# hsp-iit/online-detection

Measured on AMD Instinct MI355X. Metric: FALKON fit+infer samples/sec (N=1e6 D=1024 M=1e4), higher is better.
Workload: dtype f32-accurate K_nM (X Z' as a two-term f16 split on the f16 MFMA, f32 accumulate) stored as 24-bit fixed point (step 2^-24) + f64 solver (preconditioner: K_MM, T and T^-1 in f64; the products of the A factor, which only preconditions, at f32 accuracy on the f16 MFMA)

## Files before the change

### include/odx.h

```cpp
#ifndef ODX_H
#define ODX_H
#include <stdint.h>
#ifdef __cplusplus
extern "C" {
#endif

#define ODX_OK 0
#define ODX_ERR_INVALID (-1)
#define ODX_ERR_HIP (-2)
#define ODX_ERR_UNSUPPORTED (-3)
#define ODX_ERR_WORKSPACE (-4)

typedef void* odx_stream_t;

const char* odx_last_error_string(void);
int odx_version(void);
int odx_device_cus(void);
int odx_set_option(const char* name, int value);
int odx_get_option(const char* name, int* value);
int odx_option_default(const char* name, int* value);
int odx_release_helper_streams(void);
int odx_set_helper_streams(odx_stream_t s0, odx_stream_t s1);
int odx_stream_create_cu_mask(const uint32_t* mask, int words, odx_stream_t* stream);
int odx_stream_destroy(odx_stream_t stream);
// ... 112 lines not shown
                                  void* workspace, int64_t workspace_bytes, odx_stream_t stream);
int64_t odx_knm_fwd_bwd_q_workspace_bytes(int64_t n, int64_t M, int fmt);
int odx_knm_fwd_bwd_q(const void* K, int64_t ldk, const void* Klo, int64_t ldlo, int fmt, int64_t n, int64_t M,
                      const double* v, const double* w, double* out, void* workspace, int64_t workspace_bytes,
                      odx_stream_t stream);
int64_t odx_knm_fwd_bwd2_q_workspace_bytes(int64_t n, int64_t M, int fmt);
int odx_knm_fwd_bwd2_q(const void* K, int64_t ldk, const void* Klo, int64_t ldlo, int fmt, int64_t n, int64_t M,
                       const double* v, const double* v2, double* out, double* out2, void* workspace,
                       int64_t workspace_bytes, odx_stream_t stream);
int odx_knm_fwd_bwd_q_t(const void* K, int64_t ldk, const void* Klo, int64_t ldlo, int fmt, int64_t n, int64_t M,
                        const double* v, const double* w, double* out, double* t_out, void* workspace,
                        int64_t workspace_bytes, odx_stream_t stream);
int odx_knm_fwd_bwd2_q_t(const void* K, int64_t ldk, const void* Klo, int64_t ldlo, int fmt, int64_t n, int64_t M,
                         const double* v, const double* v2, double* out, double* out2, double* t_out, void* workspace,
                         int64_t workspace_bytes, odx_stream_t stream);
int odx_knm_fwd_bwd_q_cols_t(const void* K, int64_t ldk, const void* Klo, int64_t ldlo, int fmt, int64_t n, int64_t M,
                             const double* v, const double* w, double* out, double* t_out, void* workspace,
                             int64_t workspace_bytes, int64_t Mv, const int32_t* col_of, const int32_t* start,
                             const int32_t* pos, odx_stream_t stream);
int odx_knm_fwd_bwd2_q_cols_t(const void* K, int64_t ldk, const void* Klo, int64_t ldlo, int fmt, int64_t n, int64_t M,
                              const double* v, const double* v2, double* out, double* out2, double* t_out, void* workspace,
                              int64_t workspace_bytes, int64_t Mv, const int32_t* col_of, const int32_t* start,
                              const int32_t* pos, odx_stream_t stream);
int odx_cols_fold_f64(const double* v, int64_t Mv, const int32_t* start, const int32_t* pos, int64_t M, double* out,
                      odx_stream_t stream);
int odx_cols_expand_f64(const double* x, int64_t M, const int32_t* col_of, int64_t Mv, double* out, odx_stream_t stream);
int64_t odx_knm_fwd_bwdn_q_workspace_bytes(int64_t n, int64_t M, int fmt, int nv);
int odx_knm_fwd_bwdn_q(const void* K, int64_t ldk, const void* Klo, int64_t ldlo, int fmt, int64_t n, int64_t M, int nv,
                       const double* V, int64_t ldv, double* out, int64_t ldo, void* workspace, int64_t workspace_bytes,
                       odx_stream_t stream);
int64_t odx_knm_fwd_bwdn_q_rw_workspace_bytes(int64_t n, int64_t M, int fmt, int nv);
int odx_knm_fwd_bwdn_q_rw(const void* K, int64_t ldk, const void* Klo, int64_t ldlo, int fmt, int64_t n, int64_t M, int nv,
                          const double* V, int64_t ldv, const double* D, int64_t ldd, const int32_t* wrow, double* out,
                          int64_t ldo, double* T_out, int64_t ldt, void* workspace, int64_t workspace_bytes,
                          odx_stream_t stream);
int64_t odx_knm_bwdn_q_workspace_bytes(int64_t n, int64_t M, int fmt, int nv);
int odx_knm_bwdn_q(const void* K, int64_t ldk, const void* Klo, int64_t ldlo, int fmt, int64_t n, int64_t M, int nv,
                   const double* W, int64_t ldw, double* out, int64_t ldo, void* workspace, int64_t workspace_bytes,
                   odx_stream_t stream);
int64_t odx_knm_fwdn_q_workspace_bytes(int64_t n, int64_t M, int fmt, int nv);
int odx_knm_fwdn_q(const void* K, int64_t ldk, const void* Klo, int64_t ldlo, int fmt, int64_t n, int64_t M, int nv,
                   const double* V, int64_t ldv, double* T, int64_t ldt, void* workspace, int64_t workspace_bytes,
                   odx_stream_t stream);
int odx_knm_mv(const void* K, int64_t ldk, const void* Klo, int64_t ldlo, int fmt, int64_t n, int64_t M, const double* alpha,
               float* out, int64_t ldo, odx_stream_t stream);
int64_t odx_gauss_ktk_stream_h2_rows(int64_t M, int D);
// ... 263 lines not shown
```

### online-detection_amd/csrc/knm_pass_q.hip

```cpp
#include <algorithm>
#include <stdlib.h>

#include "odx_internal.h"
#include "knm_q.h"

namespace odx {

template <int NT, int CH, int R, int NV, int FMT, int WPE>
__device__ __forceinline__ void knm_passq_body(const unsigned short* __restrict__ Khi, int64_t ldk,
                                               const unsigned char* __restrict__ Klo, int64_t ldlo, int64_t n,
                                               int64_t M, const double* __restrict__ v1, const double* __restrict__ v2,
                                               const double* __restrict__ w, double* __restrict__ slab, int64_t slab_ld,
                                               double* __restrict__ t_out, int wg, int nwg, int64_t Mv = 0,
                                               const int* __restrict__ cstart = nullptr, const int* __restrict__ cpos = nullptr) {
  constexpr int NW = NT / 64;
  constexpr int CW = QCW;
  extern __shared__ __attribute__((aligned(16))) double vsq[];
  __shared__ double red[2][NW][NV * R];
  const int tid = threadIdx.x, lane = tid & 63, wave = tid >> 6;
  const int nchunk = (int)((M + CW - 1) / CW);
  const int vcap = (nchunk + 1) * CW;
  const int64_t nblk = (n + R - 1) / R;
  const double vscale = FMT == QF_U24 ? 5.9604644775390625e-08 : 1.0;
  for (int i = tid; i < vcap; i += NT) {
// ... 156 lines not shown
  knm_passq_body<NT, CH, R, NV, FMT, WPE>(Khi, ldk, Klo, ldlo, n, M, v1, v2, w, slab, slab_ld, t_out, (int)blockIdx.x, (int)gridDim.x, Mv,
                                          cstart, cpos);
}

struct PassBatchQ {
  const unsigned short* Khi[ODX_MAX_ZBATCH];
  const unsigned char* Klo[ODX_MAX_ZBATCH];
  int64_t ldk[ODX_MAX_ZBATCH];
  int64_t ldlo[ODX_MAX_ZBATCH];
  int64_t n[ODX_MAX_ZBATCH];
  int M[ODX_MAX_ZBATCH];
  int grid[ODX_MAX_ZBATCH];
};

template <int NT, int CH, int R, int FMT, int WPE = (NT >= 1024 ? 4 : 2)>
__global__ __launch_bounds__(NT, WPE) void knm_passq_batched_kernel(PassBatchQ pb, const double* __restrict__ v, int64_t vstride,
                                                                    double* __restrict__ slab, int64_t slab_ld, int64_t slab_stride) {
  const int b = blockIdx.y;
  if ((int)blockIdx.x >= pb.grid[b]) return;
  knm_passq_body<NT, CH, R, 1, FMT, WPE>(pb.Khi[b], pb.ldk[b], pb.Klo[b], pb.ldlo[b], pb.n[b], pb.M[b], v + (int64_t)b * vstride, nullptr,
                                         nullptr, slab + (int64_t)b * slab_stride, slab_ld, nullptr, (int)blockIdx.x, pb.grid[b]);
}

template <int CH, int R, int FMT>
__device__ __forceinline__ void knm_passq_stag_body(const unsigned short* __restrict__ Khi, int64_t ldk,
                                                    const unsigned char* __restrict__ Klo, int64_t ldlo, int64_t n,
                                                    int64_t M, const double* __restrict__ v1,
                                                    const double* __restrict__ w, double* __restrict__ slab,
                                                    int64_t slab_ld, double* __restrict__ t_out, int wg, int nwg,
                                                    int64_t Mv = 0, const int* __restrict__ cstart = nullptr,
                                                    const int* __restrict__ cpos = nullptr) {
  constexpr int NT = 256, CW = QCW;
  extern __shared__ __attribute__((aligned(16))) double vsq[];
  __shared__ double red[2][2][4][R];
  const int tid = threadIdx.x, lane = tid & 63;
  const int h = __builtin_amdgcn_readfirstlane(tid >> 8), hw = __builtin_amdgcn_readfirstlane((tid >> 6) & 3);
  const int ht = tid & 255;
  const int nchunk = (int)((M + CW - 1) / CW);
  constexpr int vcap = CH * NT * CW;
  const int64_t nblk = (n + R - 1) / R;
  const double vscale = FMT == QF_U24 ? 5.9604644775390625e-08 : 1.0;
  for (int i = tid; i < vcap; i += 512) vsq[i] = (v1 != nullptr && i < M) ? q_v_entry(v1, i, Mv, cstart, cpos) * vscale : 0.0;
  const int voff_hi = ht * (2 * CW), voff_lo = ht * CW;
  double acc[CH][CW];
#pragma unroll
  for (int c = 0; c < CH; ++c)
#pragma unroll
    for (int e = 0; e < CW; ++e) acc[c][e] = 0.0;
  QChunk<FMT, CW> kr[R][CH];
  const int rowb_hi = (int)ldk * 2, rowb_lo = (int)ldlo;
  __amdgpu_buffer_rsrc_t rs_hi, rs_lo;
  int rows_open = R;
  auto open_block = [&](int64_t blk) {
    const int64_t row0 = blk * R;
    rows_open = (int)(n - row0 < R ? n - row0 : R);
    rs_hi = __builtin_amdgcn_make_buffer_rsrc(const_cast<unsigned short*>(Khi + row0 * ldk), (short)0, rows_open * rowb_hi, 0x00020000);
    if (FMT == QF_U24)
      rs_lo = __builtin_amdgcn_make_buffer_rsrc(const_cast<unsigned char*>(Klo + row0 * ldlo), (short)0, rows_open * rowb_lo, 0x00020000);
  };
  auto load_block = [&](int c) {
#pragma unroll
    for (int r = 0; r < R; ++r) {
      const int rr = r < rows_open ? r : rows_open - 1;
      const u32x2q th = __builtin_amdgcn_raw_buffer_load_b64(rs_hi, voff_hi, rr * rowb_hi + c * (NT * 2 * CW), 0);
      kr[r][c].hi[0] = th[0], kr[r][c].hi[1] = th[1];
      if (FMT == QF_U24) kr[r][c].lo[0] = __builtin_amdgcn_raw_buffer_load_b32(rs_lo, voff_lo, rr * rowb_lo + c * (NT * CW), 0);
    }
  };
  __shared__ unsigned int arrived[2];
  if (tid < 2) arrived[tid] = 0u;
  const int64_t first = 2 * (int64_t)wg + h, step = 2 * (int64_t)nwg;
// ... 53 lines not shown
      pp ^= 1;
#pragma unroll
      for (int c = 0; c < CH; ++c)
#pragma unroll
        for (int r = 0; r < R; ++r) {
          asm volatile("" : "+v"(kr[r][c].hi[0]));
          asm volatile("" : "+v"(kr[r][c].hi[1]));
          if (FMT == QF_U24) asm volatile("" : "+v"(kr[r][c].lo[0]));
        }
    }
    if (t_out != nullptr && hw == 0) {
      if (lane == 0) {
#pragma unroll
        for (int r = 0; r < R; ++r)
          if (blk * R + r < n) t_out[blk * R + r] = t[r];
      }
    }
#pragma unroll
    for (int r = 0; r < R; ++r) {
      const int64_t row = blk * R + r;
      if (row >= n) t[r] = 0.0;
      else if (w != nullptr) t[r] += w[row];
    }
    const bool more = k + 1 < mine;
    if (more) open_block(blk + step);
#pragma unroll
    for (int c = 0; c < CH; ++c) {
#pragma unroll
      for (int r = 0; r < R; ++r)
#pragma unroll
        for (int e = 0; e < CW; ++e) acc[c][e] = fma(q_entry<FMT, CW>(kr[r][c], e), t[r], acc[c][e]);
      load_block(c);
      __builtin_amdgcn_sched_barrier(0);
    }
  }
  double* my = slab + (2 * (int64_t)wg + h) * slab_ld;
#pragma unroll
  for (int c = 0; c < CH; ++c) {
    const int ch = ht + c * NT;
    if (ch < nchunk) {
#pragma unroll
      for (int e = 0; e < CW; ++e)
        if ((int64_t)ch * CW + e < slab_ld) my[(int64_t)ch * CW + e] = acc[c][e] * vscale;
    }
  }
}

template <int CH, int R, int FMT>
__global__ __launch_bounds__(512, 2) void knm_passq_stag_kernel(const unsigned short* __restrict__ Khi, int64_t ldk,
                                                                const unsigned char* __restrict__ Klo, int64_t ldlo, int64_t n,
                                                                int64_t M, const double* __restrict__ v1,
                                                                const double* __restrict__ w, double* __restrict__ slab,
                                                                int64_t slab_ld, double* __restrict__ t_out, int64_t Mv,
                                                                const int* __restrict__ cstart, const int* __restrict__ cpos) {
  knm_passq_stag_body<CH, R, FMT>(Khi, ldk, Klo, ldlo, n, M, v1, w, slab, slab_ld, t_out, (int)blockIdx.x, (int)gridDim.x, Mv, cstart, cpos);
}

template <int CH, int R, int FMT>
__global__ __launch_bounds__(512, 2) void knm_passq_stag_batched_kernel(PassBatchQ pb, const double* __restrict__ v, int64_t vstride,
                                                                        double* __restrict__ slab, int64_t slab_ld,
                                                                        int64_t slab_stride) {
  const int b = blockIdx.y;
  if ((int)blockIdx.x >= pb.grid[b]) return;
  knm_passq_stag_body<CH, R, FMT>(pb.Khi[b], pb.ldk[b], pb.Klo[b], pb.ldlo[b], pb.n[b], pb.M[b], v + (int64_t)b * vstride, nullptr,
                                  slab + (int64_t)b * slab_stride, slab_ld, nullptr, (int)blockIdx.x, pb.grid[b]);
}

struct QCfg {
  int nt, ch, r, wg_per_cu;
};

static bool pick_qcfg(int64_t M, int nv, int fmt, QCfg* cfg) {
  const int64_t chunks = (M + 3) / 4;
  if (nv == 1) {
    if (chunks <= 256) { *cfg = {256, 1, 16, 2}; return true; }
    if (chunks <= 512) { *cfg = {0, 2, 8, 2}; return true; }
    if (chunks <= 1024) { *cfg = {0, 4, 4, 2}; return true; }
    if (chunks <= 2048) { *cfg = {256, 8, 3, 2}; return true; }
    if (chunks <= 2560) { *cfg = {0, 10, 2, 1}; return true; }
    if (chunks <= 3072) { *cfg = {512, 6, 4, 1}; return true; }
    if (chunks <= 5110) { *cfg = {1024, 5, 1, 1}; return true; }
    return false;
  }
  if (chunks <= 1024 || chunks > 2560) return false;
  if (chunks <= 2048) *cfg = {512, 4, 2, 1};
  else *cfg = {512, 5, 2, 1};
  const int64_t lds = 2 * (chunks + 1) * 4 * 8 + 2 * (cfg->nt / 64) * cfg->r * 2 * 8 + 64;
  return lds <= 163840;
// ... 246 lines not shown
  ODX_PROPAGATE(require_workspace("odx_knm_fwd_bwd2_q", workspace, workspace_bytes, 2 * (int64_t)grid * slab_ld * (int64_t)sizeof(double)));
  double* slab = static_cast<double*>(workspace);
  const size_t lds = (size_t)(2 * (slab_ld + 4) * sizeof(double));
  ODX_PROPAGATE(q_dispatch(q_block(K, ldk, Klo, ldlo, fmt, n, M), [&](auto f, const QBlock& b) {
    return dispatch_passq<2, decltype(f)::value>(cfg, b, grid, lds, s, v, v2, nullptr, slab, slab_ld, t_out, cm);
  }));
  ODX_CHECK_LAUNCH("odx_knm_fwd_bwd2_q");
  if (cm.on()) return slab_reduce_cols_f64(slab, slab_ld, grid, 2, M, cm.Mv, cm.col_of, out, out2, s);
  return slab_reduce2_f64(slab, slab_ld, grid, M, out, out2, s);
}

extern "C" int odx_knm_fwd_bwd2_q(const void* K, int64_t ldk, const void* Klo, int64_t ldlo, int fmt, int64_t n, int64_t M,
                                  const double* v, const double* v2, double* out, double* out2, void* workspace,
                                  int64_t workspace_bytes, odx_stream_t stream) {
  return knm_fwd_bwd2_q_impl(K, ldk, Klo, ldlo, fmt, n, M, v, v2, out, out2, nullptr, workspace, workspace_bytes, stream);
}

extern "C" int odx_knm_fwd_bwd2_q_t(const void* K, int64_t ldk, const void* Klo, int64_t ldlo, int fmt, int64_t n, int64_t M,
                                    const double* v, const double* v2, double* out, double* out2, double* t_out, void* workspace,
                                    int64_t workspace_bytes, odx_stream_t stream) {
  return knm_fwd_bwd2_q_impl(K, ldk, Klo, ldlo, fmt, n, M, v, v2, out, out2, t_out, workspace, workspace_bytes, stream);
}

extern "C" int odx_knm_fwd_bwd_q_cols_t(const void* K, int64_t ldk, const void* Klo, int64_t ldlo, int fmt, int64_t n, int64_t M,
                                        const double* v, const double* w, double* out, double* t_out, void* workspace,
                                        int64_t workspace_bytes, int64_t Mv, const int32_t* col_of, const int32_t* start,
                                        const int32_t* pos, odx_stream_t stream) {
  ODX_REQUIRE(t_out == nullptr || v != nullptr, "odx_knm_fwd_bwd_q_cols_t: t_out needs v");
  const QCols cm = {Mv, col_of, start, pos};
  ODX_PROPAGATE(check_q_cols("odx_knm_fwd_bwd_q_cols_t", cm, M));
  return knm_fwd_bwd_q_impl(K, ldk, Klo, ldlo, fmt, n, M, v, w, out, t_out, workspace, workspace_bytes, stream, cm);
}

extern "C" int odx_knm_fwd_bwd2_q_cols_t(const void* K, int64_t ldk, const void* Klo, int64_t ldlo, int fmt, int64_t n, int64_t M,
                                         const double* v, const double* v2, double* out, double* out2, double* t_out,
                                         void* workspace, int64_t workspace_bytes, int64_t Mv, const int32_t* col_of,
                                         const int32_t* start, const int32_t* pos, odx_stream_t stream) {
  const QCols cm = {Mv, col_of, start, pos};
  ODX_PROPAGATE(check_q_cols("odx_knm_fwd_bwd2_q_cols_t", cm, M));
  return knm_fwd_bwd2_q_impl(K, ldk, Klo, ldlo, fmt, n, M, v, v2, out, out2, t_out, workspace, workspace_bytes, stream, cm);
}
```

### online-detection_amd/odx/hip.py

```python
import ctypes
import os

_LIB = None
_LIB_PATH = os.environ.get("ODX_LIB_PATH") or os.path.join(os.path.dirname(os.path.abspath(__file__)), "lib", "libodx.so")

ODX_OK = 0
KNM_F32, KNM_U24, KNM_BF16 = 0, 1, 2
KNM_CODE = {"f32": KNM_F32, "u24": KNM_U24, "bf16": KNM_BF16}
KERNEL_GAUSS, KERNEL_MATERN32, KERNEL_MATERN52 = 0, 1, 2
STREAM_MAX_VECTORS = 16
GRID_MAX_SIGMAS = 4
GEMM_LOWER_ONLY, GEMM_A_UPPER, GEMM_B_UPPER, GEMM_A_LOWER, GEMM_B_LOWER, GEMM_STORE_T = 1, 2, 4, 8, 16, 32


class OdxUnavailable(RuntimeError):
    pass


class OdxError(RuntimeError):
    pass


_vp, _i64, _i32, _f64, _f32 = ctypes.c_void_p, ctypes.c_int64, ctypes.c_int, ctypes.c_double, ctypes.c_float

# ... 61 lines not shown
                                 _i64, _vp]),
    "odx_falkon_cg_batched_workspace_bytes": (_i64, [_i32, _vp, _vp]),
    "odx_falkon_cg_batched_f64": (_i32, [_i32, _vp, _vp, _vp, _vp, _vp, _i64, _i64, _i64, _vp, _i64, _vp, _f64, _i32, _i32, _f64, _f64,
                                         _vp, _vp, _i64, _vp]),
    "odx_falkon_cg_batched_q_workspace_bytes": (_i64, [_i32, _vp, _vp, _i32]),
    "odx_falkon_cg_batched_q_f64": (_i32, [_i32, _vp, _vp, _vp, _vp, _i32, _vp, _vp, _vp, _i64, _i64, _i64, _vp, _i64, _vp, _f64, _i32, _i32,
                                           _f64, _f64, _vp, _vp, _i64, _vp]),
    "odx_knm_fwd_bwd_workspace_bytes": (_i64, [_i64, _i64]),
    "odx_set_pass_reserved_cus": (_i32, [_i32]),
    "odx_knm_fwd_bwd": (_i32, [_vp, _i64, _i64, _i64, _vp, _vp, _vp, _vp, _i64, _vp]),
    "odx_knm_fwd_bwd2_workspace_bytes": (_i64, [_i64, _i64]),
    "odx_knm_fwd_bwd2": (_i32, [_vp, _i64, _i64, _i64, _vp, _vp, _vp, _vp, _vp, _i64, _vp]),
    "odx_knm_ld": (_i64, [_i64, _i32]),
    "odx_knm_bytes": (_i64, [_i64, _i64, _i32]),
    "odx_gauss_knm_h2_store": (_i32, [_vp, _i64, _vp, _vp, _i64, _vp, _i64, _vp, _vp, _i64, _i32, _f64, _i32, _vp, _i64, _vp, _i64,
                                      _vp, _vp, _vp, _i64, _vp]),
    "odx_knm_fwd_bwd_t": (_i32, [_vp, _i64, _i64, _i64, _vp, _vp, _vp, _vp, _vp, _i64, _vp]),
    "odx_knm_fwd_bwd2_t": (_i32, [_vp, _i64, _i64, _i64, _vp, _vp, _vp, _vp, _vp, _vp, _i64, _vp]),
    "odx_knm_fwd_bwd_q_t": (_i32, [_vp, _i64, _vp, _i64, _i32, _i64, _i64, _vp, _vp, _vp, _vp, _vp, _i64, _vp]),
    "odx_knm_fwd_bwd2_q_t": (_i32, [_vp, _i64, _vp, _i64, _i32, _i64, _i64, _vp, _vp, _vp, _vp, _vp, _vp, _i64, _vp]),
    "odx_knm_fwd_bwd_q_cols_t": (_i32, [_vp, _i64, _vp, _i64, _i32, _i64, _i64, _vp, _vp, _vp, _vp, _vp, _i64, _i64, _vp, _vp, _vp, _vp]),
    "odx_knm_fwd_bwd2_q_cols_t": (_i32, [_vp, _i64, _vp, _i64, _i32, _i64, _i64, _vp, _vp, _vp, _vp, _vp, _vp, _i64, _i64, _vp, _vp, _vp,
                                         _vp]),
    "odx_cols_fold_f64": (_i32, [_vp, _i64, _vp, _vp, _i64, _vp, _vp]),
    "odx_cols_expand_f64": (_i32, [_vp, _i64, _vp, _i64, _vp, _vp]),
    "odx_cg_scores_axpy_f64": (_i32, [_vp, _vp, _vp, _i64, _vp]),
    "odx_cg_scores_store_f32": (_i32, [_vp, _i64, _vp, _i64, _vp]),
    "odx_knm_fwd_bwd_q_workspace_bytes": (_i64, [_i64, _i64, _i32]),
    "odx_knm_fwd_bwd_q": (_i32, [_vp, _i64, _vp, _i64, _i32, _i64, _i64, _vp, _vp, _vp, _vp, _i64, _vp]),
    "odx_knm_fwd_bwd2_q_workspace_bytes": (_i64, [_i64, _i64, _i32]),
    "odx_knm_fwd_bwd2_q": (_i32, [_vp, _i64, _vp, _i64, _i32, _i64, _i64, _vp, _vp, _vp, _vp, _vp, _i64, _vp]),
    "odx_knm_fwd_bwdn_q_workspace_bytes": (_i64, [_i64, _i64, _i32, _i32]),
    "odx_knm_fwd_bwdn_q": (_i32, [_vp, _i64, _vp, _i64, _i32, _i64, _i64, _i32, _vp, _i64, _vp, _i64, _vp, _i64, _vp]),
    "odx_knm_fwd_bwdn_q_rw_workspace_bytes": (_i64, [_i64, _i64, _i32, _i32]),
    "odx_knm_fwd_bwdn_q_rw": (_i32, [_vp, _i64, _vp, _i64, _i32, _i64, _i64, _i32, _vp, _i64, _vp, _i64, _vp, _vp, _i64, _vp, _i64,
                                     _vp, _i64, _vp]),
    "odx_knm_bwdn_q_workspace_bytes": (_i64, [_i64, _i64, _i32, _i32]),
    "odx_knm_bwdn_q": (_i32, [_vp, _i64, _vp, _i64, _i32, _i64, _i64, _i32, _vp, _i64, _vp, _i64, _vp, _i64, _vp]),
    "odx_knm_fwdn_q_workspace_bytes": (_i64, [_i64, _i64, _i32, _i32]),
    "odx_knm_fwdn_q": (_i32, [_vp, _i64, _vp, _i64, _i32, _i64, _i64, _i32, _vp, _i64, _vp, _i64, _vp, _i64, _vp]),
    "odx_knm_mv": (_i32, [_vp, _i64, _vp, _i64, _i32, _i64, _i64, _vp, _vp, _i64, _vp]),
    "odx_gauss_ktk_stream_h2_rows": (_i64, [_i64, _i32]),
    "odx_gauss_ktk_stream_h2_workspace_bytes": (_i64, [_i64, _i64, _i32]),
    "odx_gauss_ktk_stream_h2": (_i32, [_vp, _i64, _vp, _vp, _i64, _vp, _i64, _vp, _vp, _i64, _i32, _f64, _vp, _vp, _vp, _vp, _vp, _vp,
                                       _i64, _vp]),
    "odx_gauss_ktk_stream_h2n_rows": (_i64, [_i64, _i32]),
# ... 134 lines not shown
```

### online-detection_amd/odx/knm_path.py

```python
import ctypes

import torch

from . import hip


def _p(t):
    return ctypes.c_void_p(t.data_ptr()) if t is not None else ctypes.c_void_p(0)


def _compact(K):
    return K.fmt in hip.KNM_CODE and K.fmt != "f32"


def _qblock(K):
    return _p(K.K), K.ld, _p(K.lo), K.ld, hip.KNM_CODE[K.fmt]


def _mapped(K):
    return getattr(K, "cmap", None)


def _vlen(K):
    return K.Mv if _mapped(K) is not None else K.M
# ... 93 lines not shown
            return False
        return K.fmt == "stream" or self._ktk2_bytes(K) >= 0

    def ktk2(self, K, v1, v2, out1=None, out2=None, t_out=None):
        if t_out is not None:
            self._check_t_out(K, v1, t_out)
        if out1 is None:
            out1 = torch.empty(_vlen(K), dtype=torch.float64, device=self.device)
        if out2 is None:
            out2 = torch.empty(_vlen(K), dtype=torch.float64, device=self.device)
        if K.fmt == "stream":
            self._ktk_stream(K, v1, v2, None, out1, out2)
            return out1, out2
        vecs = (_p(v1), _p(v2), _p(out1), _p(out2), _p(t_out))
        if _compact(K) and _mapped(K) is not None:
            ws = self._pass_ws("ktk", "odx_knm_fwd_bwd2_q", K, hip.KNM_CODE[K.fmt])
            self._call("odx_knm_fwd_bwd2_q_cols_t", *_qblock(K), K.n, K.M, *vecs, _p(ws), ws.numel(), *_cols(K, self.device))
        elif _compact(K):
            ws = self._pass_ws("ktk", "odx_knm_fwd_bwd2_q", K, hip.KNM_CODE[K.fmt])
            self._call("odx_knm_fwd_bwd2_q_t", *_qblock(K), K.n, K.M, *vecs, _p(ws), ws.numel())
        else:
            ws = self._pass_ws("ktk", "odx_knm_fwd_bwd2", K)
            self._call("odx_knm_fwd_bwd2_t", *_fblock(K), K.n, K.M, *vecs, _p(ws), ws.numel())
        return out1, out2

    def _ktkn_bytes(self, K, nv):
        return self.lib.odx_knm_fwd_bwdn_q_workspace_bytes(max(K.n, 1), K.M, hip.KNM_CODE[K.fmt], nv)

    def ktkn_width(self, K):
        if _compact(K):
            for nv in (8, 4):
                if self._ktkn_bytes(K, nv) >= 0:
                    return nv
        return 2 if self.can_ktk2(K) else 1

    def ktkn_span(self, K):
        return hip.STREAM_MAX_VECTORS if K.fmt == "stream" else self.ktkn_width(K)

    def _ktkn_stream(self, K, V, out, l, g):
        F, Zf = K.F, K.Zf
        nbytes = self._pass_bytes("odx_gauss_ktk_stream_h2n", max(K.n, 1), K.M, F.D, g)
        ws = K.ring if K.ring is not None and K.ring.numel() >= nbytes else self._workspace("ktkn_stream", nbytes)
        self._call("odx_gauss_ktk_stream_h2n", _p(F.P), F.P.stride(0), _p(F.meta), _p(F.sq), K.n, _p(Zf.P), Zf.P.stride(0), _p(Zf.meta),
                   _p(Zf.sq), K.M, F.D, K.sigma, g, _p(V[l]), V.stride(0), _p(out[l]), out.stride(0), _p(ws), ws.numel())

    def _ktkn_plan(self, K, L):
# ... 223 lines not shown
```

### online-detection_amd/odx/solver.py

```python
import math
from dataclasses import dataclass

import torch


@dataclass
class SolverOptions:
    pc_epsilon: float = 1e-5
    cg_epsilon: float = 1e-7
    cg_tolerance: float = 1e-7
    cg_full_gradient_every: int = 10
    check_pivots: bool = True


_DEFERRED = None


class deferred_pivot_checks:

    def __enter__(self):
        global _DEFERRED
        self._prev, self.items = _DEFERRED, []
        _DEFERRED = self.items
        return self
# ... 56 lines not shown
class _Rows:

    def __init__(self, be, L, Mp, fold, send, recv):
        def mat():
            return be.zeros(L * Mp).view(L, Mp)
        self.B, self.X, self.R, self.Pv, self.AP, self.U, self.alpha = (mat() for _ in range(7))
        self.AX = mat() if fold else None
        self.v = (mat(), mat() if fold else None)
        self.send, self.recv = send, recv


def _slots(TT, CC, M, L=1, l=0):
    return [[(TT[j * L + l, :M], CC[j * L + l, :M]) for j in range(k)] for k in range(1, TT.shape[0] // L + 1)]


def _cg_state(be, P, lam, b0, M, io, fold, alpha=None, tk=None, scores=None):
    X, R, Pv, AP = (be.zeros(M) for _ in range(4))
    c = _CG(P, lam, be.trmv(P, "LAi", be.trmv(P, "LTi", b0)), X, R, Pv, AP, be.zeros(M) if fold else None, be.zeros(4),
            (be.zeros(M), be.zeros(M) if fold else None), io, alpha, tk, scores)
    be.cg_init(c.B, X, R, Pv, c.state)
    return c


def _pass(be, ph, K, T, C, M, t_out=None):
    kw = {} if t_out is None else {"t_out": t_out}
    if T.shape[0] == 2:
        with ph("ktk2"):
            be.ktk2(K, T[0, :M], T[1, :M], out1=C[0, :M], out2=C[1, :M], **kw)
    else:
        with ph("ktk"):
            be.ktk(K, v=T[0, :M], out=C[0, :M], **kw)


def _sum(ar, C):
    r = ar(C)
    if r is not C:
        C.copy_(r)


def _cg_run(be, cgs, exchange, n, maxiter, opt, can_fold, shared=None):
    acc = any(c.scores is not None for c in cgs)
    sh = shared
    if sh is not None:
        P, lam, L = cgs[0].P, cgs[0].lam, len(cgs)

    def Wn(*pairs, rows=False):
        k = len(pairs)
        for j, (s, _) in enumerate(pairs):
            be.trmvn(P, "LAit", getattr(sh, s), out=sh.v[j])
            be.trmvn(P, "LTit", sh.v[j], out=sh.send[j * L:(j + 1) * L])
        exchange(k, rows)
        for j, (_, out) in enumerate(pairs):
            be.trmvn(P, "LTi", sh.recv[j * L:(j + 1) * L], alpha=1.0 / n, beta=lam, Z=sh.v[j], out=sh.U)
            be.trmvn(P, "LAi", sh.U, out=getattr(sh, out))

    def W1(*pairs, rows=False):
        k = len(pairs)
        for j, (s, _) in enumerate(pairs):
            for c in cgs:
                be.trmv(c.P, "LAit", getattr(c, s), out=c.v[j])
                be.trmv(c.P, "LTit", c.v[j], out=c.io[k - 1][j][0])
        exchange(k, rows)
        for j, (_, out) in enumerate(pairs):
            for c in cgs:
                u = be.trmv(c.P, "LTi", c.io[k - 1][j][1], alpha=1.0 / n, beta=c.lam, z=c.v[j])
                be.trmv(c.P, "LAi", u, out=getattr(c, out))

    W = W1 if sh is None else Wn
    tol = opt.cg_tolerance ** 2
    for it in range(maxiter):
        full = (it + 1) % opt.cg_full_gradient_every == 0
        fold = can_fold and full and it != maxiter - 1
        if fold:
            W(("Pv", "AP"), ("X", "AX"), rows=acc)
        else:
            W(("Pv", "AP"), rows=acc)
        for c in cgs:
            be.cg_step(c.X, c.R, c.Pv, c.AP, c.state, opt.cg_epsilon, full)
        for c in cgs:
            if c.scores is not None:
                be.cg_scores_axpy(c.state, c.tk, c.scores)
        if it == maxiter - 1:
            break
        if fold:
            for c in cgs:
                be.cg_residual(c.B, c.AX, c.AP, c.state, c.R)
        elif full:
            W(("X", "AP"))
            for c in cgs:
                c.R.copy_(c.B)
                be.axpby(-1.0, c.AP, 1.0, c.R)
        for c in cgs:
            be.cg_finish(c.R, c.Pv, c.state, opt.cg_epsilon, tol)
    if sh is not None:
        be.trmvn(P, "LTit", be.trmvn(P, "LAit", sh.X, out=sh.U), out=sh.alpha)
        for l, c in enumerate(cgs):
# ... 41 lines not shown
    b0 = ar(b0)
    one_call = (shard is None and allreduce is None and phase is None and hasattr(be, "cg_solve") and not acc
                and not getattr(P, "blocks", ()))
    if one_call and getattr(K, "fmt", "f32") != "f32":
        one_call = bool(hasattr(be, "cg_batched_supported") and getattr(P, "block_rows", None) is not None
                        and getattr(K, "cmap", None) is None
                        and be.cg_batched_supported([K.n], [K.M], K.fmt))
    if one_call:
        if precond_ready is not None:
            precond_ready()
            precond_ready = None
        if K.fmt != "f32":
            b0s = be.zeros((M + 1) // 2 * 2).view(1, -1)
            b0s[0, :M].copy_(b0)
            got = be.cg_solve_batched([K], [P], b0s, [n], lam, maxiter, opt)
            alpha = None if got is None else got[0, :M].clone()
        else:
            alpha = be.cg_solve(K, P, b0, n, lam, maxiter, opt)
    if one_call and alpha is not None:
        if opt.check_pivots:
            _check_pivots(be, P)
        return (alpha, K) if return_knm else alpha

    k, Mp = 2 if can_fold else 1, (M + 1) // 2 * 2
    TT, CC = be.zeros(k * Mp).view(k, Mp), be.zeros(k * Mp).view(k, Mp)

    def exchange(k, rows):
        bcast(TT if k == 2 else TT[0, :M])
        _pass(be, ph, K, TT[:k], CC[:k], M, tk if rows else None)
        _sum(ar, CC if k == 2 else CC[0, :M])

    alpha = be.zeros(M)
    cgs = []
    if owned:
        if precond_ready is not None:
            precond_ready()
        cgs.append(_cg_state(be, P, lam, b0, M, _slots(TT, CC, M), can_fold, alpha, tk, scores_out if acc else None))
    _cg_run(be, cgs, exchange, n, maxiter, opt, can_fold)
    bcast(alpha)
    return (alpha, K) if return_knm else alpha


def falkon_fit_stats(be, G, b, n, P, lam, maxiter=20, opt=None):
    opt = opt or SolverOptions()
    n = float(n)
    if not n > 0.0:
        raise ValueError("falkon_fit_stats: the statistics must hold a positive total weight, got n = %r" % (n,))
    M = P.M
    Mp = (M + 1) // 2 * 2
    TT, CC = be.zeros(2 * Mp).view(2, Mp), be.zeros(2 * Mp).view(2, Mp)

    def exchange(k, rows):
        be.symv(G, TT[:k], out=CC[:k])

    alpha = be.zeros(M)
    cgs = [_cg_state(be, P, float(lam), b[:M] / n, M, _slots(TT, CC, M), True, alpha)]
    _cg_run(be, cgs, exchange, n, maxiter, opt, True)
    return alpha


def falkon_fit_path(be, F, y, Zf, sigma, lams, maxiter=20, opt=None, n_total=None, allreduce=None, phase=None, knm_out=None,
# ... 247 lines not shown
        raise ValueError("falkon_fit_lockstep: owners must be %d distinct ranks below %d, got %r" % (B, world, owners))
    owned = rank in owners
    P = precond
    if owned and P is None:
        with ph("precond"):
            P = be.precond(Zfs[owners.index(rank)], sigma, lam, opt.pc_epsilon)
    Mp = (M + 1) // 2 * 2
    Tall, CC = ([be.zeros(world * Mp).view(world, Mp)] for _ in range(2))
    Ks = []
    for b in range(B):
        with ph("knm"):
            Ks.append(be.knm_rhs(F, Zfs[b], sigma, ys[b] * (1.0 / n), out=None if knm_outs is None else knm_outs[b],
                                 rhs_out=CC[0][owners[b], :M])[0])
    if knm_blocks is not None:
        knm_blocks.extend(Ks)
    acc = (scores_out is not None and world == 1 and B > 0 and len(scores_out) == B
           and all(scores_from_cg(be, K) for K in Ks))
    tks = None
    if acc:
        for S in scores_out:
            S.zero_()
        tks = [torch.empty_like(S) for S in scores_out]
    can_fold = B > 0 and _can_fold(be, Ks[0], M, int(n) // world)
    if can_fold:
        Tall.append(be.zeros(world * 2 * Mp).view(world, 2 * Mp))
        CC.append(be.zeros(world * 2 * Mp).view(world, 2 * Mp))
    kmax = len(Tall)
    mine, got = be.zeros(kmax * Mp).view(kmax, Mp), be.zeros(kmax * Mp).view(kmax, Mp)

    def exchange(k, rows):
        Ta, Ca = Tall[k - 1], CC[k - 1]
        shard.gather_rows(mine[:k].view(-1), Ta)
        for b in range(B):
            o = owners[b]
            _pass(be, ph, Ks[b], Ta[o].view(k, Mp), Ca[o].view(k, Mp), M, tks[b] if rows else None)
        shard.reduce_scatter_rows(Ca, got[:k].view(-1))

    shard.reduce_scatter_rows(CC[0], got[0])
    abuf = be.zeros(Mp)
    cgs = []
    if owned:
        if precond_ready is not None:
            precond_ready()
        b = owners.index(rank)
        cgs.append(_cg_state(be, P, lam, got[0, :M], M, _slots(mine, got, M), can_fold, abuf[:M],
                             tks[b] if acc else None, scores_out[b] if acc else None))
    _cg_run(be, cgs, exchange, n, maxiter, opt, can_fold)
    shard.gather_rows(abuf, Tall[0])
    return [Tall[0][owners[b], :M].clone() for b in range(B)]
```

Before: 187,400.

## Fold full-gradient second vector into a row-scores pass reusing tracked K alpha

On full-gradient CG iterations, the second K^T K product (for X) is no longer computed from a forward product. It is computed as K^T s, where s is the per-row scores vector (K alpha) that the CG already keeps up to date. A new kernel variant accumulates K^T t and K^T s in the same streaming pass, so the forward dot products for the second vector are skipped. Score tracking is now enabled even when the caller asked for none. This adds per-iteration axpy upkeep on an n-length vector, extra registers in the kernel, and a possible drift in accuracy from the accumulated scores.

Measured after the change: 189,500, median of 6. 1.01x the previous value.

```diff
diff --git a/include/odx.h b/include/odx.h
--- a/include/odx.h
+++ b/include/odx.h
@@ -158,6 +158,13 @@
                               const double* v, const double* v2, double* out, double* out2, double* t_out, void* workspace,
                               int64_t workspace_bytes, int64_t Mv, const int32_t* col_of, const int32_t* start,
                               const int32_t* pos, odx_stream_t stream);
+int odx_knm_fwd_bwd_q_rows_t(const void* K, int64_t ldk, const void* Klo, int64_t ldlo, int fmt, int64_t n, int64_t M,
+                             const double* v, const double* s, double* out1, double* out2, double* t_out, void* workspace,
+                             int64_t workspace_bytes, odx_stream_t stream);
+int odx_knm_fwd_bwd_q_rows_cols_t(const void* K, int64_t ldk, const void* Klo, int64_t ldlo, int fmt, int64_t n, int64_t M,
+                                  const double* v, const double* s, double* out1, double* out2, double* t_out,
+                                  void* workspace, int64_t workspace_bytes, int64_t Mv, const int32_t* col_of,
+                                  const int32_t* start, const int32_t* pos, odx_stream_t stream);
 int odx_cols_fold_f64(const double* v, int64_t Mv, const int32_t* start, const int32_t* pos, int64_t M, double* out,
                       odx_stream_t stream);
 int odx_cols_expand_f64(const double* x, int64_t M, const int32_t* col_of, int64_t Mv, double* out, odx_stream_t stream);
diff --git a/online-detection_amd/csrc/knm_pass_q.hip b/online-detection_amd/csrc/knm_pass_q.hip
--- a/online-detection_amd/csrc/knm_pass_q.hip
+++ b/online-detection_amd/csrc/knm_pass_q.hip
@@ -202,14 +202,15 @@
                                          nullptr, slab + (int64_t)b * slab_stride, slab_ld, nullptr, (int)blockIdx.x, pb.grid[b]);
 }
 
-template <int CH, int R, int FMT>
+template <int CH, int R, int FMT, bool ROWS = false>
 __device__ __forceinline__ void knm_passq_stag_body(const unsigned short* __restrict__ Khi, int64_t ldk,
                                                     const unsigned char* __restrict__ Klo, int64_t ldlo, int64_t n,
                                                     int64_t M, const double* __restrict__ v1,
                                                     const double* __restrict__ w, double* __restrict__ slab,
                                                     int64_t slab_ld, double* __restrict__ t_out, int wg, int nwg,
                                                     int64_t Mv = 0, const int* __restrict__ cstart = nullptr,
-                                                    const int* __restrict__ cpos = nullptr) {
+                                                    const int* __restrict__ cpos = nullptr,
+                                                    const double* __restrict__ srow = nullptr) {
   constexpr int NT = 256, CW = QCW;
   extern __shared__ __attribute__((aligned(16))) double vsq[];
   __shared__ double red[2][2][4][R];
@@ -223,10 +224,14 @@
   for (int i = tid; i < vcap; i += 512) vsq[i] = (v1 != nullptr && i < M) ? q_v_entry(v1, i, Mv, cstart, cpos) * vscale : 0.0;
   const int voff_hi = ht * (2 * CW), voff_lo = ht * CW;
   double acc[CH][CW];
+  double acs[ROWS ? CH : 1][CW];
 #pragma unroll
   for (int c = 0; c < CH; ++c)
 #pragma unroll
-    for (int e = 0; e < CW; ++e) acc[c][e] = 0.0;
+    for (int e = 0; e < CW; ++e) {
+      acc[c][e] = 0.0;
+      if (ROWS) acs[c][e] = 0.0;
+    }
   QChunk<FMT, CW> kr[R][CH];
   const int rowb_hi = (int)ldk * 2, rowb_lo = (int)ldlo;
   __amdgpu_buffer_rsrc_t rs_hi, rs_lo;
@@ -326,6 +331,9 @@
       if (row >= n) t[r] = 0.0;
       else if (w != nullptr) t[r] += w[row];
     }
+    double ts[R];
+#pragma unroll
+    for (int r = 0; r < R; ++r) ts[r] = (ROWS && blk * R + r < n) ? srow[blk * R + r] : 0.0;
     const bool more = k + 1 < mine;
     if (more) open_block(blk + step);
 #pragma unroll
@@ -333,19 +341,30 @@
 #pragma unroll
       for (int r = 0; r < R; ++r)
 #pragma unroll
-        for (int e = 0; e < CW; ++e) acc[c][e] = fma(q_entry<FMT, CW>(kr[r][c], e), t[r], acc[c][e]);
+        for (int e = 0; e < CW; ++e) {
+          const double kd = q_entry<FMT, CW>(kr[r][c], e);
+          acc[c][e] = fma(kd, t[r], acc[c][e]);
+          if (ROWS) acs[c][e] = fma(kd, ts[r], acs[c][e]);
+        }
       load_block(c);
       __builtin_amdgcn_sched_barrier(0);
     }
   }
-  double* my = slab + (2 * (int64_t)wg + h) * slab_ld;
+  double* my = slab + (2 * (int64_t)wg + h) * slab_ld * (ROWS ? 2 : 1);
 #pragma unroll
   for (int c = 0; c < CH; ++c) {
     const int ch = ht + c * NT;
     if (ch < nchunk) {
+      if (ROWS) {
+#pragma unroll
+        for (int e = 0; e < CW; ++e) asm volatile("" : "+v"(acc[c][e]), "+v"(acs[c][e]));
+      }
 #pragma unroll
       for (int e = 0; e < CW; ++e)
-        if ((int64_t)ch * CW + e < slab_ld) my[(int64_t)ch * CW + e] = acc[c][e] * vscale;
+        if ((int64_t)ch * CW + e < slab_ld) {
+          my[(int64_t)ch * CW + e] = acc[c][e] * vscale;
+          if (ROWS) my[slab_ld + (int64_t)ch * CW + e] = acs[c][e] * vscale;
+        }
     }
   }
 }
@@ -368,6 +387,15 @@
   if ((int)blockIdx.x >= pb.grid[b]) return;
   knm_passq_stag_body<CH, R, FMT>(pb.Khi[b], pb.ldk[b], pb.Klo[b], pb.ldlo[b], pb.n[b], pb.M[b], v + (int64_t)b * vstride, nullptr,
                                   slab + (int64_t)b * slab_stride, slab_ld, nullptr, (int)blockIdx.x, pb.grid[b]);
+}
+
+template <int CH, int R, int FMT>
+__global__ __launch_bounds__(512, 2) void knm_passq_rows_kernel(
+    const unsigned short* __restrict__ Khi, int64_t ldk, const unsigned char* __restrict__ Klo, int64_t ldlo, int64_t n, int64_t M,
+    const double* __restrict__ v1, const double* __restrict__ srow, double* __restrict__ slab, int64_t slab_ld,
+    double* __restrict__ t_out, int64_t Mv, const int* __restrict__ cstart, const int* __restrict__ cpos) {
+  knm_passq_stag_body<CH, R, FMT, true>(Khi, ldk, Klo, ldlo, n, M, v1, nullptr, slab, slab_ld, t_out, (int)blockIdx.x,
+                                            (int)gridDim.x, Mv, cstart, cpos, srow);
 }
 
 struct QCfg {
@@ -660,6 +688,77 @@
   return knm_fwd_bwd2_q_impl(K, ldk, Klo, ldlo, fmt, n, M, v, v2, out, out2, t_out, workspace, workspace_bytes, stream);
 }
 
+struct QRowsCfg {
+  int ch, r;
+};
+
+static bool pick_qrows_cfg(int64_t M, int fmt, QRowsCfg* cfg) {
+  QCfg two;
+  if (!pick_qcfg(M, 2, fmt, &two)) return false;
+  const int64_t chunks = (M + 3) / 4;
+  if (chunks <= 2048) *cfg = {8, 2};
+  else *cfg = {10, 1};
+  return true;
+}
+
+static int qrows_grid(const QRowsCfg& cfg, int64_t n) {
+  const int64_t pairs = ceil_div(ceil_div(n, cfg.r), 2);
+  const int64_t g = std::min<int64_t>(pass_cus(), pairs);
+  return (int)(g < 1 ? 1 : g);
+}
+
+template <int FMT>
+static int dispatch_passq_rows(const QRowsCfg& cfg, const QBlock& b, int grid, hipStream_t s, const double* v, const double* srow,
+                               double* slab, int64_t slab_ld, double* t_out, const QCols& cm) {
+#define ODX_QR(CH_, R_)                                                                                                          \
+  if (cfg.ch == CH_ && cfg.r == R_)                                                                                              \
+  return q_launch(knm_passq_rows_kernel<CH_, R_, FMT>, dim3(grid), 512, (size_t)(CH_ * 256 * 4) * sizeof(double), s, b.hi, b.ldk,     \
+                  b.lo, b.ldlo, b.n, b.M, v, srow, slab, slab_ld, t_out, cm.Mv, cm.start, cm.pos)
+  ODX_QR(8, 2);
+  ODX_QR(10, 1);
+#undef ODX_QR
+  set_error("odx_knm_fwd_bwd_q_rows: no kernel for this configuration");
+  return ODX_ERR_UNSUPPORTED;
+}
+
+static int knm_fwd_bwd_q_rows_impl(const char* who, const void* K, int64_t ldk, const void* Klo, int64_t ldlo, int fmt, int64_t n,
+                                   int64_t M, const double* v, const double* srow, double* out, double* out2, double* t_out,
+                                   void* workspace, int64_t workspace_bytes, odx_stream_t stream, const QCols& cm = QCols()) {
+  ODX_REQUIRE(M > 0 && out && out2, "%s: M <= 0 or null out", who);
+  hipStream_t s = as_stream(stream);
+  if (n <= 0) {
+    ODX_CHECK_HIP(hipMemsetAsync(out, 0, (size_t)(cm.on() ? cm.Mv : M) * sizeof(double), s));
+    ODX_CHECK_HIP(hipMemsetAsync(out2, 0, (size_t)(cm.on() ? cm.Mv : M) * sizeof(double), s));
+    return ODX_OK;
+  }
+  ODX_REQUIRE(v && srow, "%s: null v or s", who);
+  ODX_PROPAGATE(check_q_block(who, K, ldk, Klo, ldlo, fmt, M));
+  QRowsCfg cfg;
+  if (!pick_qrows_cfg(M, fmt, &cfg)) {
+    set_error("%s: M = %lld is outside the two-vector configurations", who, (long long)M);
+    return ODX_ERR_UNSUPPORTED;
+  }
+  ODX_REQUIRE((int64_t)cfg.ch * 256 * 4 >= M, "%s: configuration narrower than the block", who);
+  const int grid = qrows_grid(cfg, n);
+  const int64_t slab_ld = round_up(M, 4);
+  const int nslab = 2 * grid;
+  ODX_PROPAGATE(require_workspace(who, workspace, workspace_bytes, 2 * (int64_t)nslab * slab_ld * (int64_t)sizeof(double)));
+  double* slab = static_cast<double*>(workspace);
+  ODX_PROPAGATE(q_dispatch(q_block(K, ldk, Klo, ldlo, fmt, n, M), [&](auto f, const QBlock& b) {
+    return dispatch_passq_rows<decltype(f)::value>(cfg, b, grid, s, v, srow, slab, slab_ld, t_out, cm);
+  }));
+  ODX_CHECK_LAUNCH(who);
+  if (cm.on()) return slab_reduce_cols_f64(slab, slab_ld, nslab, 2, M, cm.Mv, cm.col_of, out, out2, s);
+  return slab_reduce2_f64(slab, slab_ld, nslab, M, out, out2, s);
+}
+
+extern "C" int odx_knm_fwd_bwd_q_rows_t(const void* K, int64_t ldk, const void* Klo, int64_t ldlo, int fmt, int64_t n, int64_t M,
+                                        const double* v, const double* s, double* out1, double* out2, double* t_out, void* workspace,
+                                        int64_t workspace_bytes, odx_stream_t stream) {
+  return knm_fwd_bwd_q_rows_impl("odx_knm_fwd_bwd_q_rows_t", K, ldk, Klo, ldlo, fmt, n, M, v, s, out1, out2, t_out, workspace,
+                                 workspace_bytes, stream);
+}
+
 extern "C" int odx_knm_fwd_bwd_q_cols_t(const void* K, int64_t ldk, const void* Klo, int64_t ldlo, int fmt, int64_t n, int64_t M,
                                         const double* v, const double* w, double* out, double* t_out, void* workspace,
                                         int64_t workspace_bytes, int64_t Mv, const int32_t* col_of, const int32_t* start,
@@ -678,3 +777,13 @@
   ODX_PROPAGATE(check_q_cols("odx_knm_fwd_bwd2_q_cols_t", cm, M));
   return knm_fwd_bwd2_q_impl(K, ldk, Klo, ldlo, fmt, n, M, v, v2, out, out2, t_out, workspace, workspace_bytes, stream, cm);
 }
+
+extern "C" int odx_knm_fwd_bwd_q_rows_cols_t(const void* K, int64_t ldk, const void* Klo, int64_t ldlo, int fmt, int64_t n, int64_t M,
+                                             const double* v, const double* s, double* out1, double* out2, double* t_out,
+                                             void* workspace, int64_t workspace_bytes, int64_t Mv, const int32_t* col_of,
+                                             const int32_t* start, const int32_t* pos, odx_stream_t stream) {
+  const QCols cm = {Mv, col_of, start, pos};
+  ODX_PROPAGATE(check_q_cols("odx_knm_fwd_bwd_q_rows_cols_t", cm, M));
+  return knm_fwd_bwd_q_rows_impl("odx_knm_fwd_bwd_q_rows_cols_t", K, ldk, Klo, ldlo, fmt, n, M, v, s, out1, out2, t_out, workspace,
+                                 workspace_bytes, stream, cm);
+}
diff --git a/online-detection_amd/odx/hip.py b/online-detection_amd/odx/hip.py
--- a/online-detection_amd/odx/hip.py
+++ b/online-detection_amd/odx/hip.py
@@ -107,6 +107,9 @@
     "odx_knm_fwd_bwd_q_cols_t": (_i32, [_vp, _i64, _vp, _i64, _i32, _i64, _i64, _vp, _vp, _vp, _vp, _vp, _i64, _i64, _vp, _vp, _vp, _vp]),
     "odx_knm_fwd_bwd2_q_cols_t": (_i32, [_vp, _i64, _vp, _i64, _i32, _i64, _i64, _vp, _vp, _vp, _vp, _vp, _vp, _i64, _i64, _vp, _vp, _vp,
                                          _vp]),
+    "odx_knm_fwd_bwd_q_rows_t": (_i32, [_vp, _i64, _vp, _i64, _i32, _i64, _i64, _vp, _vp, _vp, _vp, _vp, _vp, _i64, _vp]),
+    "odx_knm_fwd_bwd_q_rows_cols_t": (_i32, [_vp, _i64, _vp, _i64, _i32, _i64, _i64, _vp, _vp, _vp, _vp, _vp, _vp, _i64, _i64, _vp, _vp,
+                                             _vp, _vp]),
     "odx_cols_fold_f64": (_i32, [_vp, _i64, _vp, _vp, _i64, _vp, _vp]),
     "odx_cols_expand_f64": (_i32, [_vp, _i64, _vp, _i64, _vp, _vp]),
     "odx_cg_scores_axpy_f64": (_i32, [_vp, _vp, _vp, _i64, _vp]),
diff --git a/online-detection_amd/odx/knm_path.py b/online-detection_amd/odx/knm_path.py
--- a/online-detection_amd/odx/knm_path.py
+++ b/online-detection_amd/odx/knm_path.py
@@ -139,6 +139,30 @@
         else:
             ws = self._pass_ws("ktk", "odx_knm_fwd_bwd2", K)
             self._call("odx_knm_fwd_bwd2_t", *_fblock(K), K.n, K.M, *vecs, _p(ws), ws.numel())
+        return out1, out2
+
+    fold_rows = True
+
+    def can_ktk_rows(self, K):
+        return bool(self.fold_rows and K.fmt != "stream" and _compact(K) and self.can_ktk2(K))
+
+    def ktk_rows(self, K, v, s, out1=None, out2=None, t_out=None):
+        if not _compact(K):
+            raise ValueError("ktk_rows: compact stored blocks only (u24 / bf16), got %r" % (K.fmt,))
+        if s is None or s.dtype != torch.float64 or s.numel() != K.n or not s.is_contiguous():
+            raise ValueError("ktk_rows: s must be a contiguous f64 vector of the block's %d rows" % K.n)
+        if t_out is not None:
+            self._check_t_out(K, v, t_out)
+        if out1 is None:
+            out1 = torch.empty(_vlen(K), dtype=torch.float64, device=self.device)
+        if out2 is None:
+            out2 = torch.empty(_vlen(K), dtype=torch.float64, device=self.device)
+        ws = self._workspace("ktk", 2 * self._pass_bytes("odx_knm_fwd_bwd2_q", max(K.n, 1), K.M, hip.KNM_CODE[K.fmt]))
+        vecs = (_p(v), _p(s), _p(out1), _p(out2), _p(t_out))
+        if _mapped(K) is not None:
+            self._call("odx_knm_fwd_bwd_q_rows_cols_t", *_qblock(K), K.n, K.M, *vecs, _p(ws), ws.numel(), *_cols(K, self.device))
+        else:
+            self._call("odx_knm_fwd_bwd_q_rows_t", *_qblock(K), K.n, K.M, *vecs, _p(ws), ws.numel())
         return out1, out2
 
     def _ktkn_bytes(self, K, nv):
diff --git a/online-detection_amd/odx/solver.py b/online-detection_amd/odx/solver.py
--- a/online-detection_amd/odx/solver.py
+++ b/online-detection_amd/odx/solver.py
@@ -102,9 +102,12 @@
     return c
 
 
-def _pass(be, ph, K, T, C, M, t_out=None):
+def _pass(be, ph, K, T, C, M, t_out=None, s=None):
     kw = {} if t_out is None else {"t_out": t_out}
-    if T.shape[0] == 2:
+    if s is not None:
+        with ph("ktk2"):
+            be.ktk_rows(K, T[0, :M], s, out1=C[0, :M], out2=C[1, :M], **kw)
+    elif T.shape[0] == 2:
         with ph("ktk2"):
             be.ktk2(K, T[0, :M], T[1, :M], out1=C[0, :M], out2=C[1, :M], **kw)
     else:
@@ -118,7 +121,11 @@
         C.copy_(r)
 
 
-def _cg_run(be, cgs, exchange, n, maxiter, opt, can_fold, shared=None):
+def _fold_rows(be, Ks):
+    return bool(hasattr(be, "ktk_rows") and Ks and all(be.can_ktk_rows(K) for K in Ks))
+
+
+def _cg_run(be, cgs, exchange, n, maxiter, opt, can_fold, shared=None, fold_rows=False):
     acc = any(c.scores is not None for c in cgs)
     sh = shared
     if sh is not None:
@@ -134,24 +141,31 @@
             be.trmvn(P, "LTi", sh.recv[j * L:(j + 1) * L], alpha=1.0 / n, beta=lam, Z=sh.v[j], out=sh.U)
             be.trmvn(P, "LAi", sh.U, out=getattr(sh, out))
 
-    def W1(*pairs, rows=False):
+    def W1(*pairs, rows=False, srows=False):
         k = len(pairs)
         for j, (s, _) in enumerate(pairs):
             for c in cgs:
                 be.trmv(c.P, "LAit", getattr(c, s), out=c.v[j])
-                be.trmv(c.P, "LTit", c.v[j], out=c.io[k - 1][j][0])
-        exchange(k, rows)
+                if not (srows and j == 1):
+                    be.trmv(c.P, "LTit", c.v[j], out=c.io[k - 1][j][0])
+        if srows:
+            exchange(k, rows, True)
+        else:
+            exchange(k, rows)
         for j, (_, out) in enumerate(pairs):
             for c in cgs:
                 u = be.trmv(c.P, "LTi", c.io[k - 1][j][1], alpha=1.0 / n, beta=c.lam, z=c.v[j])
                 be.trmv(c.P, "LAi", u, out=getattr(c, out))
 
     W = W1 if sh is None else Wn
+    fold_rows = bool(fold_rows and sh is None and all(c.scores is not None for c in cgs))
     tol = opt.cg_tolerance ** 2
     for it in range(maxiter):
         full = (it + 1) % opt.cg_full_gradient_every == 0
         fold = can_fold and full and it != maxiter - 1
-        if fold:
+        if fold and fold_rows:
+            W(("Pv", "AP"), ("X", "AX"), rows=acc, srows=True)
+        elif fold:
             W(("Pv", "AP"), ("X", "AX"), rows=acc)
         else:
             W(("Pv", "AP"), rows=acc)
@@ -239,12 +253,17 @@
             _check_pivots(be, P)
         return (alpha, K) if return_knm else alpha
 
+    fold_rows = bool(can_fold and (shard is None or owner is None) and scores_from_cg(be, K) and _fold_rows(be, [K]))
+    if fold_rows and not acc:
+        acc, scores_out = True, be.zeros(K.n)
+        tk = torch.empty_like(scores_out)
+
     k, Mp = 2 if can_fold else 1, (M + 1) // 2 * 2
     TT, CC = be.zeros(k * Mp).view(k, Mp), be.zeros(k * Mp).view(k, Mp)
 
-    def exchange(k, rows):
-        bcast(TT if k == 2 else TT[0, :M])
-        _pass(be, ph, K, TT[:k], CC[:k], M, tk if rows else None)
+    def exchange(k, rows, srows=False):
+        bcast(TT if k == 2 and not srows else TT[0, :M])
+        _pass(be, ph, K, TT[:k], CC[:k], M, tk if rows else None, scores_out if srows else None)
         _sum(ar, CC if k == 2 else CC[0, :M])
 
     alpha = be.zeros(M)
@@ -253,7 +272,7 @@
         if precond_ready is not None:
             precond_ready()
         cgs.append(_cg_state(be, P, lam, b0, M, _slots(TT, CC, M), can_fold, alpha, tk, scores_out if acc else None))
-    _cg_run(be, cgs, exchange, n, maxiter, opt, can_fold)
+    _cg_run(be, cgs, exchange, n, maxiter, opt, can_fold, fold_rows=fold_rows)
     bcast(alpha)
     return (alpha, K) if return_knm else alpha
 
@@ -547,18 +566,23 @@
             S.zero_()
         tks = [torch.empty_like(S) for S in scores_out]
     can_fold = B > 0 and _can_fold(be, Ks[0], M, int(n) // world)
+    fold_rows = bool(can_fold and world == 1 and all(scores_from_cg(be, K) for K in Ks) and _fold_rows(be, Ks))
+    if fold_rows and not acc:
+        acc, scores_out = True, [be.zeros(K.n) for K in Ks]
+        tks = [torch.empty_like(S) for S in scores_out]
     if can_fold:
         Tall.append(be.zeros(world * 2 * Mp).view(world, 2 * Mp))
         CC.append(be.zeros(world * 2 * Mp).view(world, 2 * Mp))
     kmax = len(Tall)
     mine, got = be.zeros(kmax * Mp).view(kmax, Mp), be.zeros(kmax * Mp).view(kmax, Mp)
 
-    def exchange(k, rows):
+    def exchange(k, rows, srows=False):
         Ta, Ca = Tall[k - 1], CC[k - 1]
         shard.gather_rows(mine[:k].view(-1), Ta)
         for b in range(B):
             o = owners[b]
-            _pass(be, ph, Ks[b], Ta[o].view(k, Mp), Ca[o].view(k, Mp), M, tks[b] if rows else None)
+            _pass(be, ph, Ks[b], Ta[o].view(k, Mp), Ca[o].view(k, Mp), M, tks[b] if rows else None,
+                  scores_out[b] if srows else None)
         shard.reduce_scatter_rows(Ca, got[:k].view(-1))
 
     shard.reduce_scatter_rows(CC[0], got[0])
@@ -570,6 +594,6 @@
         b = owners.index(rank)
         cgs.append(_cg_state(be, P, lam, got[0, :M], M, _slots(mine, got, M), can_fold, abuf[:M],
                              tks[b] if acc else None, scores_out[b] if acc else None))
-    _cg_run(be, cgs, exchange, n, maxiter, opt, can_fold)
+    _cg_run(be, cgs, exchange, n, maxiter, opt, can_fold, fold_rows=fold_rows)
     shard.gather_rows(abuf, Tall[0])
     return [Tall[0][owners[b], :M].clone() for b in range(B)]
```
